# ClashLuke/LocAtE

Measured on AMD Instinct MI355X. Metric: images/sec (G+D step) 64x64 bs=64, higher is better.
Workload: dtype f32 (contractions fp32-faithful on the matrix cores: 2 x scaled fp16 operand pieces / 3 MFMAs per slice where the operand's largest magnitude comes with it, else 3 x bf16 pieces / 6 MFMAs; fp32 accumulate); 1 GPU; LocAtE G+D step, 64x64 RGB, batch 64 per GPU (the fp32 variant - the reference's own precision - of BASELINE.json configs[1]: 64x64 RGB bs 64), self/feature attention at 16x16 and 64x64, random-init weights; global_batch=64, image_size=64, parallelism=dp1, launch=hipGraph replay, G-step generator pass on a second stream

## Files before the change

locate_amd/csrc/conv.hip:

```cpp
#include "igemm.h"

template <int WGM, int WGN, int TM, int TN>
__global__ void __launch_bounds__(256) conv_igemm_kernel(const IgParams p) {
    constexpr int BK = IG_BK;
    constexpr int BM = WGM * TM * 32;
    constexpr int BN = WGN * TN * 32;
    constexpr int KPT = BK * BN / 256;
    constexpr int A_F4 = BK * BM / 4;
    constexpr int A_PT = (A_F4 + 255) / 256;
    static_assert(WGM * WGN == 4, "four waves");
    static_assert(BN % 64 == 0 && KPT == 8, "one 8-row group of the offset table per thread and step");
    static_assert(BK <= IG_TAIL, "panel tail shorter than the prefetch distance (one stage beyond the last)");

    __shared__ __attribute__((aligned(16))) float As[2][BK][BM];
    __shared__ __attribute__((aligned(16))) float Bs[2][BK][BN];

    int bx, by, bz;
    xcd_tile(bx, by, bz, p.tile_nphase);
    const int zphase = bz / p.ksplit, zsplit = bz - zphase * p.ksplit;
    const IgPhase& ph = p.ph[zphase];
    const int N = p.B * ph.QH * ph.QW;
    const int n0 = bx * BN;
    const int m0 = by * BM;
    if (n0 >= N) return;

    const int tid = threadIdx.x, lane = tid & 63, wid = tid >> 6;
    const int wm = wid / WGN, wn = wid % WGN;

    const int ncol = tid % BN;
    const int kgrp = __builtin_amdgcn_readfirstlane(tid / BN);
    const GatherCol gc = gather_setup(p, ph, n0 + ncol, N);
    float col_scale[TN];
    igemm_col_scales<WGM, WGN, TM, TN>(p, ph, col_scale, N, n0, wn, lane);

// ... 95 lines not shown
__global__ void __launch_bounds__(64 * NW, (NW == 8 ? 1 : (WGM * TM > 4 ? 2 : ((WGM * TM * TN <= IG_FOUR_BLOCKS_TILES && WGM * TM * TN >= IG_FOUR_BLOCKS_MIN && NP <= 2) ? 4 : 3)))) conv_igemm_bx6_kernel(const IgParams p) {
    constexpr int BK = 4 * NW, KB = BK / 8, KS = BK / 16, NT = 64 * NW;
    constexpr int BM = WGM * TM * 32;
    constexpr int BN = WGN * TN * 32;
    static_assert(NW == 4 || NW == 8, "four or eight waves");
    static_assert(WGM * WGN == NW, "wave grid");
    static_assert(BN == 128 && KB * BN == NT, "one gathered fragment (k-block) per thread and stage");
    static_assert(KB * BM <= 2 * NT, "at most two weight fragments per thread and stage");
    static_assert(B6_BK == 16, "the host's split-K accounting counts 16-deep steps");
    constexpr bool A2 = KB * BM > NT;
    static_assert(2 * BK <= IG_TAIL && (IG_TAIL % 8) == 0, "panel tail shorter than the prefetch distance");

    constexpr int A_U4 = 2 * NP * KB * BM, B_U4 = 2 * NP * KB * BN;
    constexpr int EPI_U4 = (NW * 32 * 33 + 8 + 3) / 4;
    constexpr int SMEM_U4 = A_U4 + B_U4 > EPI_U4 ? A_U4 + B_U4 : EPI_U4;
    __shared__ uint4 smem[SMEM_U4];
    uint4 (*As)[NP][KB][BM] = reinterpret_cast<uint4 (*)[NP][KB][BM]>(smem);
    uint4 (*Bs)[NP][KB][BN] = reinterpret_cast<uint4 (*)[NP][KB][BN]>(smem + A_U4);

    int bx, by, bz;
    xcd_tile(bx, by, bz, p.tile_nphase);
    const int zphase = bz / p.ksplit, zsplit = bz - zphase * p.ksplit;
    const IgPhase& ph = p.ph[zphase];
    const int N = p.B * ph.QH * ph.QW;
    const int n0 = bx * BN;
    const int m0 = by * BM;
    if (n0 >= N) return;

    const int tid = threadIdx.x, lane = tid & 63, wid = tid >> 6;
    const int wm = wid / WGN, wn = wid % WGN;

    const int ncol = tid % BN;
    const int kgrp = __builtin_amdgcn_readfirstlane(tid / BN);
    const GatherCol gc = gather_setup(p, ph, n0 + ncol, N);
    float col_scale[TN];
    igemm_col_scales<WGM, WGN, TM, TN>(p, ph, col_scale, N, n0, wn, lane);
    float b_scale = 1.0f, a_unscale = 1.0f, b_unscale = 1.0f;
    if constexpr (NP == 2) {
        const int kb_ = f16_scale_exp(absmax_read(p.b_absmax));
        const int ka_ = f16_scale_exp(__builtin_amdgcn_readfirstlane(*ph.a_absmax));
        b_scale = pow2f(kb_);
        unscale_pair(ka_, kb_, a_unscale, b_unscale);
    }

    f32x16 acc[TM][TN];
#pragma unroll
    for (int i = 0; i < TM; ++i)
#pragma unroll
        for (int j = 0; j < TN; ++j)
#pragma unroll
            for (int r = 0; r < 16; ++r) acc[i][j][r] = 0.0f;

    const int total_steps = ph.Kpad / BK;
    const int per_split = (total_steps + p.ksplit - 1) / p.ksplit;
    const int step0 = zsplit * per_split;
    int nsteps = total_steps - step0;
    if (nsteps > per_split) nsteps = per_split;
    if (nsteps < 0) nsteps = 0;

    const bool a_thread = KB * BM == NT || tid < KB * BM;
    const int a_kb = a_thread ? tid / BM : 0, a_m = a_thread ? tid % BM : 0;
    const uint4* ap = ph.w3 + (long long)(step0 * KB + a_kb) * ph.ld + (m0 + a_m);
    const long long a_step = (long long)KB * ph.ld, a_plane = ph.w3_plane;
    const bool b_thread = A2 && tid + NT < KB * BM;
    const int b_kb = b_thread ? (tid + NT) / BM : 0, b_m = b_thread ? (tid + NT) % BM : 0;
    const uint4* bp = ph.w3 + (long long)(step0 * KB + b_kb) * ph.ld + (m0 + b_m);
    int kidx = step0 * BK + kgrp * 8;

    uint4 areg0, areg1, areg2;
    uint4 areg3, areg4, areg5;
    float breg[8];
    i32x8 offs = *reinterpret_cast<const i32x8*>(ph.koff + __builtin_amdgcn_readfirstlane(kidx));
    unsigned long long taps = *reinterpret_cast<const unsigned long long*>(ph.ktap + __builtin_amdgcn_readfirstlane(kidx));
    auto issue_loads = [&]() {
        areg0 = ap[0];
        if constexpr (NP >= 2) areg1 = ap[a_plane];
        if constexpr (NP == 3) areg2 = ap[2 * a_plane];
        ap += a_step;
        if constexpr (A2) {
            areg3 = bp[0];
            if constexpr (NP >= 2) areg4 = bp[a_plane];
            if constexpr (NP == 3) areg5 = bp[2 * a_plane];
            bp += a_step;
        }
#pragma unroll
        for (int j = 0; j < 8; ++j) breg[j] = gather_load(gc, offs[j], (unsigned)(taps >> (8 * j)) & 31u);
        kidx += BK;
        const int ks = __builtin_amdgcn_readfirstlane(kidx);
// ... 26 lines not shown
            float v[8];
#pragma unroll
            for (int j = 0; j < 8; ++j) v[j] = breg[j];
            split3_trunc_x8(v, h, m, l);
            Bs[buf][0][kgrp][ncol] = h;
            Bs[buf][NP - 2][kgrp][ncol] = m;
            Bs[buf][NP - 1][kgrp][ncol] = l;
        } else {
            bf16x8 h;
#pragma unroll
            for (int j = 0; j < 8; ++j) h[j] = (__bf16)breg[j];
            Bs[buf][0][kgrp][ncol] = *reinterpret_cast<uint4*>(&h);
        }
    };

    if (nsteps > 0) {
        issue_loads();
        store_tiles(0);
        issue_loads();
    }
    __syncthreads();
    const int lrow = lane >> 5, lcol = lane & 31;
    constexpr int PROD = NP == 3 ? 6 : (NP == 2 ? 3 : 1);
    constexpr int NMF = TM * TN * PROD, HALF = KS == 1 ? NMF / 2 : NMF;
    using frag_t = typename std::conditional<NP == 2, f16x8, bf16x8>::type;
    for (int s = 0; s < nsteps; ++s) {
        const int buf = s & 1;
        frag_t a[TM][NP], b[TN][NP];
        auto fragments = [&](int ksub) {
#pragma unroll
            for (int i = 0; i < TM; ++i)
#pragma unroll
                for (int q = 0; q < NP; ++q) a[i][q] = *reinterpret_cast<const frag_t*>(&As[buf][q][2 * ksub + lrow][(wm * TM + i) * 32 + lcol]);
#pragma unroll
            for (int j = 0; j < TN; ++j)
// ... 107 lines not shown
                    for (int f = 0; f < HB; ++f)
                        v[zz][f] = __builtin_amdgcn_raw_buffer_load_b128(srs, (int)(t0 + (unsigned)(z0 + zz) * zstride + (unsigned)((h0 + f) * NT * 16)), 0, 16);
#pragma unroll
                for (int zz = 0; zz < ZB; ++zz)
#pragma unroll
                    for (int f = 0; f < HB; ++f) {
                        const int g = h0 + f, i = g / (TN * 4), j = (g / 4) % TN, q = g % 4;
#pragma unroll
                        for (int e = 0; e < 4; ++e) acc[i][j][4 * q + e] += __uint_as_float(v[zz][f][e]);
                    }
            }
        }
        __syncthreads();
        combined = true;
    }
    igemm_epilogue<WGM, WGN, TM, TN>(p, ph, acc, col_scale, N, n0, m0, combined ? 0 : zsplit, wm, wn, lane, stage, p.ksplit > 1 && !combined);
}

__global__ void __launch_bounds__(256) igemm_slab_reduce_kernel(const float* __restrict__ slab, float* __restrict__ out,
                                                                const float* __restrict__ bias, const float* __restrict__ scale,
                                                                int scale_bg, int scale_stride, int B, int M, int plane,
                                                                long long out_bs, long long slab_stride, int ksplit,
                                                                float* __restrict__ act_out, long long act_bs,
                                                                const float* __restrict__ mul_pre, long long mul_bs,
                                                                unsigned* __restrict__ out_absmax) {
    const unsigned per_b = (unsigned)M * (unsigned)plane;
    const unsigned total = (unsigned)B * per_b;
    const unsigned stride = gridDim.x * blockDim.x;
    const DivU32 dpb(per_b), dpl((unsigned)plane);
    float am = 0.0f;
    for (unsigned i = blockIdx.x * blockDim.x + threadIdx.x; i < total; i += stride) {
// ... 279 lines not shown
    igemm_slab_reduce_kernel<<<stream_grid(p.slab_stride, 256), 256, 0, st>>>(p.slab, p.out, p.bias, p.scale, p.scale_bg, p.scale_stride, p.B, p.M, p.OH * p.OW,
                                                                              p.out_bs, p.slab_stride, p.ksplit, p.act_out, p.act_bs, p.mul_pre, p.mul_bs, p.out_absmax);
}

template <int NP>
static void launch_bx6(const IgParams& p, dim3 grid, int bm, bool w8, hipStream_t st) {
    if (w8) {
        if (bm == 128) conv_igemm_bx6_kernel<2, 4, 2, 1, NP, 8><<<grid, 512, 0, st>>>(p);
        else conv_igemm_bx6_kernel<2, 4, 1, 1, NP, 8><<<grid, 512, 0, st>>>(p);
        return;
    }
    with_tile<true>(bm, [&](auto t) { using T = decltype(t); conv_igemm_bx6_kernel<T::wgm, T::wgn, T::tm, T::tn, NP><<<grid, 256, 0, st>>>(p); });
}

static int launch_igemm(IgParams& p, int nmax, void* slab_ws, unsigned* counters, hipStream_t st, const char* who) {
    p.tile_nphase = (path_disabled("phasefast") || (long long)p.OH * p.OW < 1024) ? 1 : p.nphase;
    if (p.win) return launch_win_igemm(p, nmax, slab_ws, counters, st, who);
    if (skinny_ok(p)) {
        p.ksplit = 1;
        launch_skinny(p, st);
        LOCATE_LAUNCH_CHECK(who);
        return LOCATE_OK;
    }
    if (pointwise_ok(p)) {
        p.ksplit = 1;
        launch_pointwise(p, st);
        LOCATE_LAUNCH_CHECK(who);
        return LOCATE_OK;
    }
    const int bm = igemm_bm(p.M, nmax, p.nphase);
// ... 442 lines not shown
```

locate_amd/csrc/convfp8.hip:

```cpp
#include "igemm.h"

__device__ __forceinline__ uint4 quant_fp8x16(const float (&v)[16], float sc) {
    unsigned w[4];
#pragma unroll
    for (int q = 0; q < 4; ++q) {
        int t = 0;
        t = __builtin_amdgcn_cvt_pk_fp8_f32(v[4 * q + 0] * sc, v[4 * q + 1] * sc, t, false);
        t = __builtin_amdgcn_cvt_pk_fp8_f32(v[4 * q + 2] * sc, v[4 * q + 3] * sc, t, true);
        w[q] = (unsigned)t;
    }
    return make_uint4(w[0], w[1], w[2], w[3]);
}

template <int WGM, int WGN, int TM, int TN>
__global__ void __launch_bounds__(256, (WGM * TM > 4 ? 2 : 3)) conv_igemm_fp8_kernel(const IgParams p) {
    constexpr int BK = 32, KB = 2, NT = 256, NW = 4;
    constexpr int BM = WGM * TM * 32;
    constexpr int BN = WGN * TN * 32;
    static_assert(WGM * WGN == NW && BN == 128 && KB * BN == NT, "one gathered chunk (16 k) per thread and stage");
    static_assert(KB * BM <= 2 * NT, "at most two weight chunks per thread and stage");
    constexpr bool A2 = KB * BM > NT;
    static_assert(2 * BK <= IG_TAIL, "panel tail shorter than the prefetch distance");
    constexpr int A_U4 = 2 * KB * BM, B_U4 = 2 * KB * BN;
    constexpr int EPI_U4 = (NW * 32 * 33 + 8 + 3) / 4;
    constexpr int SMEM_U4 = A_U4 + B_U4 > EPI_U4 ? A_U4 + B_U4 : EPI_U4;
    __shared__ uint4 smem[SMEM_U4];
    uint4 (*As)[KB][BM] = reinterpret_cast<uint4 (*)[KB][BM]>(smem);
    uint4 (*Bs)[KB][BN] = reinterpret_cast<uint4 (*)[KB][BN]>(smem + A_U4);

    int bx, by, bz;
    xcd_tile(bx, by, bz, p.tile_nphase);
    const int zphase = bz / p.ksplit, zsplit = bz - zphase * p.ksplit;
    const IgPhase& ph = p.ph[zphase];
    const int N = p.B * ph.QH * ph.QW;
    const int n0 = bx * BN;
    const int m0 = by * BM;
    if (n0 >= N) return;

    const int tid = threadIdx.x, lane = tid & 63, wid = tid >> 6;
    const int wm = wid / WGN, wn = wid % WGN;
    const int ncol = tid % BN;
    const int kgrp = __builtin_amdgcn_readfirstlane(tid / BN);
    const GatherCol gc = gather_setup(p, ph, n0 + ncol, N);
    float col_scale[TN];
    igemm_col_scales<WGM, WGN, TM, TN>(p, ph, col_scale, N, n0, wn, lane);
    const int kb_ = f8_scale_exp(absmax_read(p.b_absmax));
    const int ka_ = f8_scale_exp(__builtin_amdgcn_readfirstlane(*ph.a_absmax));
// ... 174 lines not shown
```

locate_amd/csrc/convwgrad.hip:

```cpp
#include "igemm.h"

#define WG_BK 32

struct WgParams {
    const float* x;
    const float* gy;
    float* slab;
    long long x_bs, gy_bs;
    unsigned x_bytes;
    int B, C, H, W, M, OH, OW, KH, KW, stride, pad_h, pad_w;
    int R;
    int N;
    int chunk;
    int zper, Ng;
    unsigned q_mul, ow_mul;
    int q_s1, q_s2, ow_s1, ow_s2;
    int gscale_bg, gscale_stride;
    float* direct_out;
    const float* w_ref;
    const float* inv_scale;
    double* partial;
    const unsigned* x_absmax;
    const unsigned* g_absmax;
};


template <int WGM, int WGN, int TM, int TN>
__device__ __forceinline__ void wgrad_epilogue(const WgParams& p, f32x16 (&acc)[TM][TN], int r0, int m0, int wm, int wn, int lane,
                                               int wid, int tid) {
    const int lrow = lane >> 5, lcol = lane & 31;
    __shared__ double red[4];
    const bool direct = p.direct_out != nullptr;
    float* dst = direct ? p.direct_out : p.slab + (long long)blockIdx.z * p.M * p.R;
    const float sc = (direct && p.inv_scale && p.gscale_bg == 0) ? p.inv_scale[0] : 1.0f;
    double dot = 0.0;
    const bool want_dot = direct && p.w_ref != nullptr;
#pragma unroll
    for (int j = 0; j < TN; ++j) {
        const int r = r0 + (wn * TN + j) * 32 + lcol;
// ... 17 lines not shown
                if (r_ok && m < p.M) dst[(long long)m * p.R + r] = v * sc;
            }
            dot += (double)part;
        }
    }
    if (direct && p.partial) {
        dot = wave_sum_d(dot);
        if (lane == 0) red[wid] = dot;
        __syncthreads();
        if (tid == 0) p.partial[blockIdx.y * gridDim.x + blockIdx.x] = (red[0] + red[1]) + (red[2] + red[3]);
    }
}

template <int WGM, int WGN, int TM, int TN>
__global__ void __launch_bounds__(256) conv_wgrad_kernel(const WgParams p) {
    constexpr int BM = WGM * TM * 32;
    constexpr int BR = WGN * TN * 32;
    constexpr int G_PT = WG_BK * BM / 256;
    constexpr int X_PT = WG_BK * BR / 256;
    static_assert(WGM * WGN == 4, "four waves");

    __shared__ float Gs[2][WG_BK][BM + 1];
    __shared__ float Xs[2][WG_BK][BR + 1];
    __shared__ int rt_off[BR];
    __shared__ signed char rt_dy[BR], rt_dx[BR];

    const int tid = threadIdx.x, lane = tid & 63, wid = tid >> 6;
    const int wm = wid / WGN, wn = wid % WGN;
    const int r0 = blockIdx.x * BR, m0 = blockIdx.y * BM;
    const int taps = p.KH * p.KW;
// ... 108 lines not shown
#pragma unroll
                for (int j = 0; j < TN; ++j) acc[i][j] = __builtin_amdgcn_mfma_f32_32x32x2f32(a[i], b[j], acc[i][j], 0, 0, 0);
        }
        if (s + 1 < nsteps) store_tiles(buf ^ 1);
        __syncthreads();
    }

    wgrad_epilogue<WGM, WGN, TM, TN>(p, acc, r0, m0, wm, wn, lane, wid, tid);
}

#define WB_BK 16
#define WB_PITCH 8

template <int WGM, int WGN, int TM, int TN, int NP>
__global__ void __launch_bounds__(256, (WGM * TM > 4 ? 2 : 3)) conv_wgrad_bx6_kernel(const WgParams p) {
    constexpr int BM = WGM * TM * 32;
    constexpr int BR = WGN * TN * 32;
    constexpr int G_PT = BM / 32;
    constexpr int X_PT = BR / 32;
    static_assert(WGM * WGN == 4, "four waves");

    constexpr int NPL = NP == 4 ? 1 : NP;
    __shared__ unsigned Gs[2][NPL][NP == 4 ? 1 : BM][WB_PITCH];
    __shared__ unsigned Xs[2][NPL][NP == 4 ? 1 : BR][WB_PITCH];
    __shared__ __attribute__((aligned(16))) unsigned short G8[2][NP == 4 ? BM : 1][8];
    __shared__ __attribute__((aligned(16))) unsigned short X8[2][NP == 4 ? BR : 1][8];

    const int tid = threadIdx.x, lane = tid & 63, wid = tid >> 6;
    const int wm = wid / WGN, wn = wid % WGN;
    const int r0 = blockIdx.x * BR, m0 = blockIdx.y * BM;
// ... 436 lines not shown
}

static int wgrad_reduce_zp(int nsplit, int64_t n) {
    if (nsplit >= 64 && n < knob_int("LOCATE_ZP16_MAX_N", 1 << 12)) return 16;
    return (nsplit >= 16 && n < (1 << 20)) ? 4 : 1;
}
static int wgrad_reduce_grid(int64_t n, int nsplit) {
    const int epb = 256 / wgrad_reduce_zp(nsplit, n);
    int g = stream_grid(n, epb);
    return g > 2048 ? 2048 : g;
}

struct PwParams {
    const float* x;
    const float* gy;
    float* slab;
    const float* inv_scale;
    long long x_bs, gy_bs;
    int B, C, M, P;
    int N;
    int steps, chunk;
    int tiles_c;
    int gscale_bg, gscale_stride;
    const unsigned* x_absmax;
    const unsigned* g_absmax;
};

template <int TM, int TN, int NP>
__global__ void __launch_bounds__(256) pw_wgrad_kernel(const PwParams p) {
    __shared__ float red[3][TM * TN * 16][64];
    const int lane = threadIdx.x & 63, wid = __builtin_amdgcn_readfirstlane((int)threadIdx.x >> 6);
    const int lrow = lane >> 5, lcol = lane & 31;
    const int tm = blockIdx.y / p.tiles_c, tc = blockIdx.y - tm * p.tiles_c;
    const int m0 = tm * (TM * 32), c0 = tc * (TN * 32);
    const int z = blockIdx.x * 4 + wid;
    const int s_begin = z * p.chunk;
    int s_end = s_begin + p.chunk;
    if (s_end > p.steps) s_end = p.steps;

    float gs0 = 1.0f, gs1 = 1.0f, gs2 = 1.0f, gs3 = 1.0f;
    if (p.gscale_bg > 0) {
        const int ng = p.B / p.gscale_bg;
        gs0 = p.inv_scale[0];
        gs1 = ng > 1 ? p.inv_scale[p.gscale_stride] : 1.0f;
// ... 611 lines not shown
    if (r.kind == WG_ONEPIX) {
        const OnePix op = {g.H * g.W, g.W, g.KH, g.KW, g.pad_h, g.pad_w, g.C};
        skinny_wgrad_kernel<<<r.grid, 256, 0, st>>>(x, x_bs, gy, gy_bs, gw, w_ref, inv_scale, scale_group_batch, scale_stride,
                                                   inner_partial, g.B, g.M, g.C * g.H * g.W, op);
        LOCATE_LAUNCH_CHECK("locate_conv_wgrad(one output pixel)");
        return LOCATE_OK;
    }
    const dim3 grid = r.grid;
    if (r.kind == WG_POINTWISE) {
        const PwPlan& pq = r.pw;
        LOCATE_REQUIRE((x_bs & 3) == 0 && (gy_bs & 3) == 0 &&
                       ((reinterpret_cast<uintptr_t>(x) | reinterpret_cast<uintptr_t>(gy)) & 15) == 0,
                       "locate_conv_wgrad: narrow 1x1 layers need 16-byte aligned x / gy and batch strides that are multiples of 4");
        LOCATE_REQUIRE(workspace, "locate_conv_wgrad: the split reduction needs a workspace");
        PwParams q;
        q.x = x; q.gy = gy; q.slab = static_cast<float*>(workspace); q.x_bs = x_bs; q.gy_bs = gy_bs;
        q.B = g.B; q.C = g.C; q.M = g.M; q.P = g.H * g.W; q.N = g.B * g.H * g.W; q.steps = pq.steps; q.chunk = pq.chunk;
        q.tiles_c = pq.tiles_c;
        const bool grouped = scale_group_batch > 0;
        q.inv_scale = grouped ? inv_scale : nullptr; q.gscale_bg = scale_group_batch; q.gscale_stride = scale_stride;
        const int key = (pq.tm - 1) * 2 + (pq.tn - 1);
        q.x_absmax = static_cast<const unsigned*>(x_absmax);
        q.g_absmax = static_cast<const unsigned*>(gy_absmax);
        if (precision == 2 && x_absmax && gy_absmax && !grouped) {
            if (key == 0) pw_wgrad_kernel<1, 1, 2><<<grid, 256, 0, st>>>(q);
            else if (key == 1) pw_wgrad_kernel<1, 2, 2><<<grid, 256, 0, st>>>(q);
            else if (key == 2) pw_wgrad_kernel<2, 1, 2><<<grid, 256, 0, st>>>(q);
            else pw_wgrad_kernel<2, 2, 2><<<grid, 256, 0, st>>>(q);
        } else if (precision == 1) {
            if (key == 0) pw_wgrad_kernel<1, 1, 1><<<grid, 256, 0, st>>>(q);
            else if (key == 1) pw_wgrad_kernel<1, 2, 1><<<grid, 256, 0, st>>>(q);
            else if (key == 2) pw_wgrad_kernel<2, 1, 1><<<grid, 256, 0, st>>>(q);
            else pw_wgrad_kernel<2, 2, 1><<<grid, 256, 0, st>>>(q);
        } else {
            if (key == 0) pw_wgrad_kernel<1, 1, 3><<<grid, 256, 0, st>>>(q);
            else if (key == 1) pw_wgrad_kernel<1, 2, 3><<<grid, 256, 0, st>>>(q);
            else if (key == 2) pw_wgrad_kernel<2, 1, 3><<<grid, 256, 0, st>>>(q);
            else pw_wgrad_kernel<2, 2, 3><<<grid, 256, 0, st>>>(q);
        }
        LOCATE_LAUNCH_CHECK("locate_conv_wgrad(pointwise)");
        return reduce(q.slab, grouped ? nullptr : inv_scale, "locate_conv_wgrad(pointwise reduce)");
    }
    const int bm = r.bm, nsplit = r.nsplit, chunk = r.chunk, zper = r.zper;
    LOCATE_REQUIRE(nsplit == 1 || workspace, "locate_conv_wgrad: split reduction needs a workspace");
    WgParams p;
    p.x = x; p.gy = gy; p.slab = static_cast<float*>(workspace); p.x_bs = x_bs; p.gy_bs = gy_bs;
    p.B = g.B; p.C = g.C; p.H = g.H; p.W = g.W; p.M = g.M; p.OH = g.OH; p.OW = g.OW; p.KH = g.KH; p.KW = g.KW;
    p.stride = g.stride; p.pad_h = g.pad_h; p.pad_w = g.pad_w;
    p.R = g.C * g.KH * g.KW; p.N = g.B * g.OH * g.OW; p.chunk = chunk;
    p.zper = zper; p.Ng = gd > 1 ? p.N / gd : p.N;
    fastdiv_make((unsigned)(g.OH * g.OW), &p.q_mul, &p.q_s1, &p.q_s2);
    fastdiv_make((unsigned)g.OW, &p.ow_mul, &p.ow_s1, &p.ow_s2);
    const bool direct = nsplit == 1;
    const bool grouped = scale_group_batch > 0;
    p.gscale_bg = scale_group_batch; p.gscale_stride = scale_stride;
    p.x_absmax = static_cast<const unsigned*>(x_absmax);
    p.g_absmax = static_cast<const unsigned*>(gy_absmax);
    p.direct_out = direct ? gw : nullptr;
    p.w_ref = direct ? w_ref : nullptr;
    p.inv_scale = (direct || grouped) ? inv_scale : nullptr;
// ... 43 lines not shown
```

locate_amd/csrc/convwin.hip:

```cpp
#include "igemm.h"

typedef unsigned u32x2 __attribute__((ext_vector_type(2)));
typedef int i32x2 __attribute__((ext_vector_type(2)));
typedef int i32x4 __attribute__((ext_vector_type(4)));

template <int WGM, int WGN, int TM, int TN, int NP, int SL, int BPT>
__global__ void __launch_bounds__(256, 2) conv_win_kernel(const IgParams p) {
    constexpr int NT = 256, NW = 4, U = 2 * SL;
    constexpr int BM = WGM * TM * 32;
    constexpr int BN = WGN * TN * 32;
    static_assert(WGM * WGN == NW && (BN == 128 || BN == 256), "four waves on a 128- or 256-column tile");
    constexpr int A_CH = U * BM;
    constexpr int A_PT = (A_CH + NT - 1) / NT;
    constexpr int A_U4 = 2 * NP * A_CH;
    static_assert(2 * U <= WIN_TAIL_UNITS, "panel tail shorter than the prefetch distance");

    extern __shared__ uint4 smem[];

    int bx, by, bz;
    xcd_tile(bx, by, bz, p.tile_nphase);
    const int zphase = bz / p.ksplit, zsplit = bz - zphase * p.ksplit;
    const IgPhase& ph = p.ph[zphase];
    const int QHW = ph.QH * ph.QW;
    const int N = p.B * QHW;
    const int n0 = bx * BN;
    const int m0 = by * BM;
    if (n0 >= N) return;

    const int tid = threadIdx.x, lane = tid & 63, wid = tid >> 6;
    const int wm = wid / WGN, wn = wid % WGN;
    const int lrow = lane >> 5, lcol = lane & 31;

    const int T = ph.T, Tp = ph.win_Tp, NG = ph.win_NG;
    const int WINC = Tp == 1 ? U : 1;
    const int SP = p.win_slotsp;
    const int HW = p.H * p.W;
// ... 493 lines not shown
```

locate_amd/csrc/igemm.h:

```cpp
#pragma once
#include "common.h"
#include <cstdlib>
#include <cstring>
#include <stdlib.h>
#include <type_traits>

#ifdef LOCATE_DEBUG_KNOBS
static bool path_disabled(const char* name) {
    static const char* env = getenv("LOCATE_DISABLE");
    return env != nullptr && strstr(env, name) != nullptr;
}
static int knob_int(const char* name, int fallback) {
    const char* v = getenv(name);
    return v != nullptr ? atoi(v) : fallback;
}
#else
static constexpr bool path_disabled(const char*) { return false; }
static constexpr int knob_int(const char*, int fallback) { return fallback; }
#endif

typedef float f32x16 __attribute__((ext_vector_type(16)));

#define IG_BK 16
#define IG_KPAD 32
// ... 158 lines not shown
        ll[j] = (_Float16)(x - (float)hh[j]);
    }
    h = *reinterpret_cast<uint4*>(&hh);
    l = *reinterpret_cast<uint4*>(&ll);
}

__device__ __forceinline__ void split2_f16_pair(float v0, float v1, unsigned& h, unsigned& l) {
    typedef _Float16 f16x2 __attribute__((ext_vector_type(2)));
    f16x2 hh, ll;
    hh[0] = (_Float16)v0; hh[1] = (_Float16)v1;
    ll[0] = (_Float16)(v0 - (float)hh[0]); ll[1] = (_Float16)(v1 - (float)hh[1]);
    h = *reinterpret_cast<unsigned*>(&hh);
    l = *reinterpret_cast<unsigned*>(&ll);
}

struct IgPhase {
    const float* wp;
    const int* koff;
    const unsigned char* ktap;
    const uint4* w3;
    const unsigned* a_absmax;
    long long w3_plane;
    int K, Kpad, ld, T;
    int dmin;
    int oy0, ox0, QH, QW;
    int TW, tw_magic;
    int dy0, dys, dx0, dxs;
    int win_Tp, win_NG, win_TR, win_NI, win_WR;
    unsigned win_wrw_mul;
    int win_wrw_s1, win_wrw_s2;
    int tapc[32] __attribute__((aligned(32)));
};

struct IgParams {
    const float* in;
    float* out;
    const float* bias;
    const float* scale;
    int scale_bg;
    int scale_stride;
    long long in_bs, out_bs;
    unsigned in_bytes;
    int B, C, H, W;
    int M, OH, OW;
    int istride, ostep, nphase;
    int ksplit;
    float* slab;
    long long slab_stride;
    int precision;
    const unsigned* b_absmax;
    float* act_out = nullptr;
    long long act_bs = 0;
    const float* lat = nullptr;
    long long lat_bs = 0;
    int lat_z = 0;
    const float* mul_pre = nullptr;
    long long mul_bs = 0;
    unsigned* out_absmax = nullptr;
    int combine;
    unsigned* counters;
    int tile_nphase;
    int win;
    int win_dbg;
    int win_U, win_slotsp, win_bm, win_bn;
    IgPhase ph[4];
};

template <int WGM, int WGN, int TM, int TN>
__device__ __forceinline__ void igemm_col_scales(const IgParams& p, const IgPhase& ph, float (&col_scale)[TN], int N, int n0,
                                                 int wn, int lane) {
    const int lcol = lane & 31;
#pragma unroll
    for (int j = 0; j < TN; ++j) {
        const int nj = n0 + (wn * TN + j) * 32 + lcol;
        const int nn = nj < N ? nj : 0;
        const int b = nn / (ph.QH * ph.QW);
        col_scale[j] = p.scale ? p.scale[(p.scale_bg ? b / p.scale_bg : 0) * p.scale_stride] : 1.0f;
    }
}

template <int WGM, int WGN, int TM, int TN>
__device__ __forceinline__ void igemm_epilogue(const IgParams& p, const IgPhase& ph, f32x16 (&acc)[TM][TN],
                                               const float (&col_scale)[TN], int N, int n0, int m0, int zsplit, int wm,
                                               int wn, int lane, float* stage, bool split) {
    const int lrow = lane >> 5, lcol = lane & 31;
    const long long plane = (long long)p.OH * p.OW;
    const int iplane = (int)plane;
    if (stage != nullptr && p.nphase == 1 && p.ostep == 1 && iplane <= 16 && (iplane & (iplane - 1)) == 0 &&
        ph.QH * ph.QW == iplane) {
        const int lp = __ffs(iplane) - 1;
        const bool fused_s = !split && (p.act_out != nullptr || p.mul_pre != nullptr);
        float am_s = 0.0f;
        float* out_base = split ? p.slab + (long long)zsplit * p.slab_stride : p.out;
        const long long obs = split ? (long long)p.M * plane : p.out_bs;
#pragma unroll
        for (int i = 0; i < TM; ++i) {
            const int mt0 = m0 + (wm * TM + i) * 32;
            float bias_v[16];
#pragma unroll
            for (int r = 0; r < 16; ++r) {
                const int m = mt0 + (r & 3) + 8 * (r >> 2) + 4 * lrow;
                const bool use = p.bias != nullptr && !split && m < p.M;
                const float* bp = use ? p.bias + m : p.in;
                bias_v[r] = use ? *bp : 0.0f;
            }
#pragma unroll
            for (int j = 0; j < TN; ++j) {
                const int nt0 = n0 + (wn * TN + j) * 32;
#pragma unroll
                for (int r = 0; r < 16; ++r) {
                    const int ml = (r & 3) + 8 * (r >> 2) + 4 * lrow;
                    stage[lcol * 33 + ml] = split ? acc[i][j][r] : fmaf(acc[i][j][r], col_scale[j], bias_v[r]);
                }
                __builtin_amdgcn_fence(__ATOMIC_SEQ_CST, "wavefront");
                const int b0 = nt0 >> lp;
                if (!fused_s) {
// ... 71 lines not shown
        const int b = nn / qhw, q = nn - b * qhw;
        const int qy = q / ph.QW, qx = q - qy * ph.QW;
        const long long pix = (long long)(ph.oy0 + qy * p.ostep) * p.OW + (ph.ox0 + qx * p.ostep);
        const float* o = split ? p.slab + (long long)zsplit * p.slab_stride + (long long)b * p.M * plane + pix
                               : p.out + (long long)b * p.out_bs + pix;
        optr[j] = nj < N ? o : nullptr;
        xoff[j] = (long long)b * ((p.mul_pre ? p.mul_bs : p.act_bs) - p.out_bs);
    }
    float am = 0.0f;
#pragma unroll
    for (int i = 0; i < TM; ++i) {
        float bias_v[16];
#pragma unroll
        for (int r = 0; r < 16; ++r) {
            const int m = m0 + (wm * TM + i) * 32 + (r & 3) + 8 * (r >> 2) + 4 * lrow;
            const bool use = p.bias != nullptr && !split && m < p.M;
            const float* bp = use ? p.bias + m : p.in;
            bias_v[r] = use ? *bp : 0.0f;
        }
#pragma unroll
        for (int j = 0; j < TN; ++j) {
            float* o = const_cast<float*>(optr[j]);
            if (o == nullptr) continue;
            if (!fused) {
#pragma unroll
                for (int r = 0; r < 16; ++r) {
                    const int m = m0 + (wm * TM + i) * 32 + (r & 3) + 8 * (r >> 2) + 4 * lrow;
                    if (m < p.M) o[(long long)m * plane] = split ? acc[i][j][r] : fmaf(acc[i][j][r], col_scale[j], bias_v[r]);
                }
            } else if (p.mul_pre != nullptr) {
// ... 67 lines not shown
            const int th = (t * ph.tw_magic) >> 16, tw = t - th * ph.TW;
            const bool ok = (unsigned)(iy0 + ph.dy0 + ph.dys * th) < (unsigned)p.H &&
                            (unsigned)(ix0 + ph.dx0 + ph.dxs * tw) < (unsigned)p.W;
            inside |= (ok ? 1u : 0u) << t;
        }
    }
    g.outside = ~inside;
    return g;
}

__device__ __forceinline__ float gather_load(const GatherCol& g, int soff, unsigned tap) {
    const unsigned vo = ((g.outside << (31u - tap)) & 0x80000000u) | g.lane_off;
    return __builtin_bit_cast(float, __builtin_amdgcn_raw_buffer_load_b32(g.rsrc, (int)vo, soff, 0));
}

typedef int i32x8 __attribute__((ext_vector_type(8)));
typedef unsigned u32x4 __attribute__((ext_vector_type(4)));


__device__ __forceinline__ int fastdiv(int n, unsigned mul, int s1, int s2) {
    const unsigned t = __umulhi((unsigned)n, mul);
    return (int)((t + (((unsigned)n - t) >> s1)) >> s2);
}
static void fastdiv_make(unsigned d, unsigned* mul, int* s1, int* s2) {
    if (d <= 1) { *mul = 0; *s1 = 0; *s2 = 0; return; }
    int l = 0;
    while ((1ull << l) < d) ++l;
    *mul = (unsigned)(((1ull << 32) * ((1ull << l) - d)) / d + 1);
    *s1 = 1; *s2 = l - 1;
}

// ... 19 lines not shown
```

Measured before the change: 7268 images/sec.

## Prefetch hot kernel-argument lines in bursts and stage bias in LDS early

Reorders the IgParams, IgPhase, WgParams and PwParams structs so the fields each prologue reads sit in the first one or two 64-byte lines. Each conv kernel now starts with an inline-asm burst of scalar loads that pulls those kernarg lines into the scalar cache at once, instead of taking serial misses. In the bx6 kernel, the offset/tap table and absmax reads are issued earlier; the b-absmax read is done one line per lane and reduced with DPP, and the bias is loaded once into LDS before the main loop instead of in the epilogue. This adds inline asm that depends on the struct layout and a small LDS allocation, with debug knobs to turn each piece off.

```diff
diff --git a/locate_amd/csrc/conv.hip b/locate_amd/csrc/conv.hip
--- a/locate_amd/csrc/conv.hip
+++ b/locate_amd/csrc/conv.hip
@@ -15,9 +15,11 @@
     __shared__ __attribute__((aligned(16))) float As[2][BK][BM];
     __shared__ __attribute__((aligned(16))) float Bs[2][BK][BN];
 
+    if (!HOT_ARGS_LAZY(p)) hot_args_burst<true>();
     int bx, by, bz;
     xcd_tile(bx, by, bz, p.tile_nphase);
     const int zphase = bz / p.ksplit, zsplit = bz - zphase * p.ksplit;
+    if (zphase > 0 && !HOT_ARGS_LAZY(p)) hot_phase_burst<2>(zphase);
     const IgPhase& ph = p.ph[zphase];
     const int N = p.B * ph.QH * ph.QW;
     const int n0 = bx * BN;
@@ -143,13 +145,18 @@
     constexpr int A_U4 = 2 * NP * KB * BM, B_U4 = 2 * NP * KB * BN;
     constexpr int EPI_U4 = (NW * 32 * 33 + 8 + 3) / 4;
     constexpr int SMEM_U4 = A_U4 + B_U4 > EPI_U4 ? A_U4 + B_U4 : EPI_U4;
-    __shared__ uint4 smem[SMEM_U4];
+    __shared__ uint4 smem[SMEM_U4 + BM / 4];
     uint4 (*As)[NP][KB][BM] = reinterpret_cast<uint4 (*)[NP][KB][BM]>(smem);
     uint4 (*Bs)[NP][KB][BN] = reinterpret_cast<uint4 (*)[NP][KB][BN]>(smem + A_U4);
-
+    float* const bias_s = reinterpret_cast<float*>(smem + SMEM_U4);
+
+    constexpr bool HOT_OK = !(NP == 1 && NW == 4 && WGM * TM * TN == 1);
+    const bool hot = HOT_OK && !HOT_EARLY_OFF(p), hot_bias = HOT_OK && !HOT_BIAS_OFF(p), hot_burst = HOT_OK && !HOT_ARGS_LAZY(p);
+    if (hot_burst) hot_args_burst<true>();
     int bx, by, bz;
     xcd_tile(bx, by, bz, p.tile_nphase);
     const int zphase = bz / p.ksplit, zsplit = bz - zphase * p.ksplit;
+    if (zphase > 0 && hot_burst) hot_phase_burst<2>(zphase);
     const IgPhase& ph = p.ph[zphase];
     const int N = p.B * ph.QH * ph.QW;
     const int n0 = bx * BN;
@@ -161,24 +168,6 @@
 
     const int ncol = tid % BN;
     const int kgrp = __builtin_amdgcn_readfirstlane(tid / BN);
-    const GatherCol gc = gather_setup(p, ph, n0 + ncol, N);
-    float col_scale[TN];
-    igemm_col_scales<WGM, WGN, TM, TN>(p, ph, col_scale, N, n0, wn, lane);
-    float b_scale = 1.0f, a_unscale = 1.0f, b_unscale = 1.0f;
-    if constexpr (NP == 2) {
-        const int kb_ = f16_scale_exp(absmax_read(p.b_absmax));
-        const int ka_ = f16_scale_exp(__builtin_amdgcn_readfirstlane(*ph.a_absmax));
-        b_scale = pow2f(kb_);
-        unscale_pair(ka_, kb_, a_unscale, b_unscale);
-    }
-
-    f32x16 acc[TM][TN];
-#pragma unroll
-    for (int i = 0; i < TM; ++i)
-#pragma unroll
-        for (int j = 0; j < TN; ++j)
-#pragma unroll
-            for (int r = 0; r < 16; ++r) acc[i][j][r] = 0.0f;
 
     const int total_steps = ph.Kpad / BK;
     const int per_split = (total_steps + p.ksplit - 1) / p.ksplit;
@@ -186,6 +175,37 @@
     int nsteps = total_steps - step0;
     if (nsteps > per_split) nsteps = per_split;
     if (nsteps < 0) nsteps = 0;
+    int kidx = step0 * BK + kgrp * 8;
+
+    i32x8 offs;
+    unsigned long long taps;
+    unsigned b_word = 0, a_word = 0;
+    if (hot) {
+        offs = *reinterpret_cast<const i32x8*>(ph.koff + __builtin_amdgcn_readfirstlane(kidx));
+        taps = *reinterpret_cast<const unsigned long long*>(ph.ktap + __builtin_amdgcn_readfirstlane(kidx));
+        if constexpr (NP == 2) {
+            b_word = p.b_absmax[AMAX_STRIDE * (tid & (AMAX_LINES - 1))];
+            a_word = *ph.a_absmax;
+        }
+    }
+    const GatherCol gc = gather_setup(p, ph, n0 + ncol, N);
+    float col_scale[TN];
+    igemm_col_scales<WGM, WGN, TM, TN>(p, ph, col_scale, N, n0, wn, lane);
+    float b_scale = 1.0f, a_unscale = 1.0f, b_unscale = 1.0f;
+    if constexpr (NP == 2) {
+        const int kb_ = f16_scale_exp(hot ? absmax_reduce_dpp(b_word) : absmax_read(p.b_absmax));
+        const int ka_ = f16_scale_exp(__builtin_amdgcn_readfirstlane(hot ? a_word : *ph.a_absmax));
+        b_scale = pow2f(kb_);
+        unscale_pair(ka_, kb_, a_unscale, b_unscale);
+    }
+
+    f32x16 acc[TM][TN];
+#pragma unroll
+    for (int i = 0; i < TM; ++i)
+#pragma unroll
+        for (int j = 0; j < TN; ++j)
+#pragma unroll
+            for (int r = 0; r < 16; ++r) acc[i][j][r] = 0.0f;
 
     const bool a_thread = KB * BM == NT || tid < KB * BM;
     const int a_kb = a_thread ? tid / BM : 0, a_m = a_thread ? tid % BM : 0;
@@ -194,13 +214,14 @@
     const bool b_thread = A2 && tid + NT < KB * BM;
     const int b_kb = b_thread ? (tid + NT) / BM : 0, b_m = b_thread ? (tid + NT) % BM : 0;
     const uint4* bp = ph.w3 + (long long)(step0 * KB + b_kb) * ph.ld + (m0 + b_m);
-    int kidx = step0 * BK + kgrp * 8;
 
     uint4 areg0, areg1, areg2;
     uint4 areg3, areg4, areg5;
     float breg[8];
-    i32x8 offs = *reinterpret_cast<const i32x8*>(ph.koff + __builtin_amdgcn_readfirstlane(kidx));
-    unsigned long long taps = *reinterpret_cast<const unsigned long long*>(ph.ktap + __builtin_amdgcn_readfirstlane(kidx));
+    if (!hot) {
+        offs = *reinterpret_cast<const i32x8*>(ph.koff + __builtin_amdgcn_readfirstlane(kidx));
+        taps = *reinterpret_cast<const unsigned long long*>(ph.ktap + __builtin_amdgcn_readfirstlane(kidx));
+    }
     auto issue_loads = [&]() {
         areg0 = ap[0];
         if constexpr (NP >= 2) areg1 = ap[a_plane];
@@ -257,11 +278,19 @@
         }
     };
 
+    float bias_r = 0.0f;
+    static_assert(BM <= NT, "one bias row per thread");
+    if (hot_bias) {
+        const bool use = p.bias != nullptr && tid < BM && m0 + tid < p.M;
+        const float* bp_ = use ? p.bias + (m0 + tid) : p.in;
+        bias_r = use ? *bp_ : 0.0f;
+    }
     if (nsteps > 0) {
         issue_loads();
         store_tiles(0);
         issue_loads();
     }
+    if (hot_bias && tid < BM) bias_s[tid] = bias_r;
     __syncthreads();
     const int lrow = lane >> 5, lcol = lane & 31;
     constexpr int PROD = NP == 3 ? 6 : (NP == 2 ? 3 : 1);
@@ -399,7 +428,8 @@
         __syncthreads();
         combined = true;
     }
-    igemm_epilogue<WGM, WGN, TM, TN>(p, ph, acc, col_scale, N, n0, m0, combined ? 0 : zsplit, wm, wn, lane, stage, p.ksplit > 1 && !combined);
+    igemm_epilogue<WGM, WGN, TM, TN>(p, ph, acc, col_scale, N, n0, m0, combined ? 0 : zsplit, wm, wn, lane, stage, p.ksplit > 1 && !combined,
+                                     hot_bias ? bias_s : nullptr);
 }
 
 __global__ void __launch_bounds__(256) igemm_slab_reduce_kernel(const float* __restrict__ slab, float* __restrict__ out,
@@ -709,6 +739,7 @@
 }
 
 static int launch_igemm(IgParams& p, int nmax, void* slab_ws, unsigned* counters, hipStream_t st, const char* who) {
+    p.lazy = (path_disabled("hotargs") ? 7 : 0) | (path_disabled("hotburst") ? 1 : 0) | (path_disabled("hotearly") ? 2 : 0) | (path_disabled("hotbias") ? 4 : 0);
     p.tile_nphase = (path_disabled("phasefast") || (long long)p.OH * p.OW < 1024) ? 1 : p.nphase;
     if (p.win) return launch_win_igemm(p, nmax, slab_ws, counters, st, who);
     if (skinny_ok(p)) {
diff --git a/locate_amd/csrc/convfp8.hip b/locate_amd/csrc/convfp8.hip
--- a/locate_amd/csrc/convfp8.hip
+++ b/locate_amd/csrc/convfp8.hip
@@ -28,9 +28,11 @@
     uint4 (*As)[KB][BM] = reinterpret_cast<uint4 (*)[KB][BM]>(smem);
     uint4 (*Bs)[KB][BN] = reinterpret_cast<uint4 (*)[KB][BN]>(smem + A_U4);
 
+    if (!HOT_ARGS_LAZY(p)) hot_args_burst<true>();
     int bx, by, bz;
     xcd_tile(bx, by, bz, p.tile_nphase);
     const int zphase = bz / p.ksplit, zsplit = bz - zphase * p.ksplit;
+    if (zphase > 0 && !HOT_ARGS_LAZY(p)) hot_phase_burst<2>(zphase);
     const IgPhase& ph = p.ph[zphase];
     const int N = p.B * ph.QH * ph.QW;
     const int n0 = bx * BN;
diff --git a/locate_amd/csrc/convwgrad.hip b/locate_amd/csrc/convwgrad.hip
--- a/locate_amd/csrc/convwgrad.hip
+++ b/locate_amd/csrc/convwgrad.hip
@@ -2,27 +2,35 @@
 
 #define WG_BK 32
 
-struct WgParams {
+struct alignas(64) WgParams {
     const float* x;
     const float* gy;
-    float* slab;
     long long x_bs, gy_bs;
+    const unsigned* x_absmax;
+    const unsigned* g_absmax;
+    const float* inv_scale;
     unsigned x_bytes;
-    int B, C, H, W, M, OH, OW, KH, KW, stride, pad_h, pad_w;
+    int B, H, W, M, OH, OW, KH, KW, stride, pad_h, pad_w;
     int R;
-    int N;
     int chunk;
     int zper, Ng;
+    int gscale_bg, gscale_stride;
     unsigned q_mul, ow_mul;
     int q_s1, q_s2, ow_s1, ow_s2;
-    int gscale_bg, gscale_stride;
+    int C;
+    int N;
+    float* slab;
     float* direct_out;
     const float* w_ref;
-    const float* inv_scale;
     double* partial;
-    const unsigned* x_absmax;
-    const unsigned* g_absmax;
+#ifdef LOCATE_DEBUG_KNOBS
+    int lazy;
+#endif
 };
+static_assert(offsetof(WgParams, x) == 0 && offsetof(WgParams, q_mul) == 128, "WgParams: the hot block is the first two 64-byte lines");
+#ifndef LOCATE_DEBUG_KNOBS
+static_assert(sizeof(WgParams) == 192, "WgParams must not grow");
+#endif
 
 
 template <int WGM, int WGN, int TM, int TN>
@@ -70,6 +78,7 @@
 
 template <int WGM, int WGN, int TM, int TN>
 __global__ void __launch_bounds__(256) conv_wgrad_kernel(const WgParams p) {
+    if (!HOT_ARGS_LAZY(p)) flat_args_burst<192>();
     constexpr int BM = WGM * TM * 32;
     constexpr int BR = WGN * TN * 32;
     constexpr int G_PT = WG_BK * BM / 256;
@@ -208,6 +217,9 @@
 
 template <int WGM, int WGN, int TM, int TN, int NP>
 __global__ void __launch_bounds__(256, (WGM * TM > 4 ? 2 : 3)) conv_wgrad_bx6_kernel(const WgParams p) {
+    if constexpr (!(NP == 1 && WGM * TM * TN == 1)) {
+        if (!HOT_ARGS_LAZY(p)) flat_args_burst<192>();
+    }
     constexpr int BM = WGM * TM * 32;
     constexpr int BR = WGN * TN * 32;
     constexpr int G_PT = BM / 32;
@@ -674,20 +686,30 @@
 struct PwParams {
     const float* x;
     const float* gy;
-    float* slab;
     const float* inv_scale;
+    const unsigned* x_absmax;
+    const unsigned* g_absmax;
     long long x_bs, gy_bs;
     int B, C, M, P;
     int N;
     int steps, chunk;
     int tiles_c;
     int gscale_bg, gscale_stride;
-    const unsigned* x_absmax;
-    const unsigned* g_absmax;
+    float* slab;
+#ifdef LOCATE_DEBUG_KNOBS
+    int lazy;
+#endif
 };
+static_assert(offsetof(PwParams, slab) == 96, "PwParams: everything the prologue reads leads");
+#ifndef LOCATE_DEBUG_KNOBS
+static_assert(sizeof(PwParams) == 104, "PwParams must not grow");
+#endif
 
 template <int TM, int TN, int NP>
 __global__ void __launch_bounds__(256) pw_wgrad_kernel(const PwParams p) {
+    if constexpr (!((NP == 1 && TM * TN == 2) || (NP == 3 && TN == 1))) {
+        if (!HOT_ARGS_LAZY(p)) flat_args_burst<104>();
+    }
     __shared__ float red[3][TM * TN * 16][64];
     const int lane = threadIdx.x & 63, wid = __builtin_amdgcn_readfirstlane((int)threadIdx.x >> 6);
     const int lrow = lane >> 5, lcol = lane & 31;
@@ -1329,6 +1351,9 @@
                        "locate_conv_wgrad: narrow 1x1 layers need 16-byte aligned x / gy and batch strides that are multiples of 4");
         LOCATE_REQUIRE(workspace, "locate_conv_wgrad: the split reduction needs a workspace");
         PwParams q;
+#ifdef LOCATE_DEBUG_KNOBS
+        q.lazy = path_disabled("hotargs") ? 1 : 0;
+#endif
         q.x = x; q.gy = gy; q.slab = static_cast<float*>(workspace); q.x_bs = x_bs; q.gy_bs = gy_bs;
         q.B = g.B; q.C = g.C; q.M = g.M; q.P = g.H * g.W; q.N = g.B * g.H * g.W; q.steps = pq.steps; q.chunk = pq.chunk;
         q.tiles_c = pq.tiles_c;
@@ -1359,6 +1384,9 @@
     const int bm = r.bm, nsplit = r.nsplit, chunk = r.chunk, zper = r.zper;
     LOCATE_REQUIRE(nsplit == 1 || workspace, "locate_conv_wgrad: split reduction needs a workspace");
     WgParams p;
+#ifdef LOCATE_DEBUG_KNOBS
+    p.lazy = path_disabled("hotargs") ? 1 : 0;
+#endif
     p.x = x; p.gy = gy; p.slab = static_cast<float*>(workspace); p.x_bs = x_bs; p.gy_bs = gy_bs;
     p.B = g.B; p.C = g.C; p.H = g.H; p.W = g.W; p.M = g.M; p.OH = g.OH; p.OW = g.OW; p.KH = g.KH; p.KW = g.KW;
     p.stride = g.stride; p.pad_h = g.pad_h; p.pad_w = g.pad_w;
diff --git a/locate_amd/csrc/convwin.hip b/locate_amd/csrc/convwin.hip
--- a/locate_amd/csrc/convwin.hip
+++ b/locate_amd/csrc/convwin.hip
@@ -17,9 +17,11 @@
 
     extern __shared__ uint4 smem[];
 
+    if (!HOT_ARGS_LAZY(p)) hot_args_burst<true>();
     int bx, by, bz;
     xcd_tile(bx, by, bz, p.tile_nphase);
     const int zphase = bz / p.ksplit, zsplit = bz - zphase * p.ksplit;
+    if (!HOT_ARGS_LAZY(p)) hot_phase_burst<5>(zphase);
     const IgPhase& ph = p.ph[zphase];
     const int QHW = ph.QH * ph.QW;
     const int N = p.B * QHW;
diff --git a/locate_amd/csrc/igemm.h b/locate_amd/csrc/igemm.h
--- a/locate_amd/csrc/igemm.h
+++ b/locate_amd/csrc/igemm.h
@@ -1,5 +1,6 @@
 #pragma once
 #include "common.h"
+#include <cstddef>
 #include <cstdlib>
 #include <cstring>
 #include <stdlib.h>
@@ -196,6 +197,7 @@
     l = *reinterpret_cast<unsigned*>(&ll);
 }
 
+#define IG_PHASE_HOT 96
 struct IgPhase {
     const float* wp;
     const int* koff;
@@ -203,50 +205,133 @@
     const uint4* w3;
     const unsigned* a_absmax;
     long long w3_plane;
-    int K, Kpad, ld, T;
+    int Kpad, ld, T;
     int dmin;
-    int oy0, ox0, QH, QW;
+    int QH, QW;
     int TW, tw_magic;
     int dy0, dys, dx0, dxs;
+    int K;
+    int oy0, ox0;
     int win_Tp, win_NG, win_TR, win_NI, win_WR;
     unsigned win_wrw_mul;
     int win_wrw_s1, win_wrw_s2;
     int tapc[32] __attribute__((aligned(32)));
 };
 
-struct IgParams {
+#define IG_HOT 128
+struct alignas(64) IgParams {
     const float* in;
     float* out;
     const float* bias;
     const float* scale;
-    int scale_bg;
-    int scale_stride;
+    const unsigned* b_absmax;
     long long in_bs, out_bs;
     unsigned in_bytes;
+    int scale_bg, scale_stride;
     int B, C, H, W;
     int M, OH, OW;
     int istride, ostep, nphase;
     int ksplit;
+    int tile_nphase;
+    int combine;
+    int win_U, win_slotsp;
     float* slab;
     long long slab_stride;
-    int precision;
-    const unsigned* b_absmax;
     float* act_out = nullptr;
     long long act_bs = 0;
+    const float* mul_pre = nullptr;
+    long long mul_bs = 0;
+    unsigned* out_absmax = nullptr;
+    unsigned* counters;
     const float* lat = nullptr;
     long long lat_bs = 0;
     int lat_z = 0;
-    const float* mul_pre = nullptr;
-    long long mul_bs = 0;
-    unsigned* out_absmax = nullptr;
-    int combine;
-    unsigned* counters;
-    int tile_nphase;
+    int precision;
     int win;
     int win_dbg;
-    int win_U, win_slotsp, win_bm, win_bn;
+    int win_bm, win_bn;
+    int lazy = 0;
     IgPhase ph[4];
 };
+static_assert(offsetof(IgParams, in) == 0 && offsetof(IgParams, slab) == IG_HOT, "IgParams: the hot block is the first two 64-byte lines");
+static_assert(offsetof(IgParams, lat) == IG_HOT + 64, "IgParams: the epilogue's fields are line 2");
+static_assert(offsetof(IgPhase, wp) == 0 && offsetof(IgPhase, K) == IG_PHASE_HOT, "IgPhase: the hot block leads");
+static_assert(offsetof(IgParams, ph) % 32 == 0 && sizeof(IgPhase) % 32 == 0 && IG_PHASE_HOT <= 96,
+              "IgPhase: a hot block of <= 96 bytes that starts on a 32-byte boundary lies inside two 64-byte lines");
+static_assert(sizeof(IgPhase) <= 288 && sizeof(IgParams) <= 1408, "the records must not grow");
+
+typedef int i32x8 __attribute__((ext_vector_type(8)));
+template <bool HIDDEN>
+__device__ __forceinline__ void hot_args_burst() {
+    const auto ka = __builtin_amdgcn_kernarg_segment_ptr();
+    int t0, t1, t2, t3, t4, t5;
+    constexpr int PH = (int)offsetof(IgParams, ph);
+    static_assert(PH % 64 == 0 && sizeof(IgParams) % 64 == 0 && IG_PHASE_HOT <= 128, "line-aligned blocks");
+    if constexpr (HIDDEN) {
+        asm volatile("s_load_dword %0, %6, 0x0\n\ts_load_dword %1, %6, %9\n\ts_load_dword %2, %6, 0x40\n\t"
+                     "s_load_dword %3, %6, %7\n\ts_load_dword %4, %6, %8\n\ts_load_dword %5, %6, 0x80\n\t"
+                     "s_waitcnt lgkmcnt(0)"
+                     : "=&s"(t0), "=&s"(t1), "=&s"(t2), "=&s"(t3), "=&s"(t4), "=&s"(t5)
+                     : "s"(ka), "i"(PH), "i"(PH + 64), "i"((int)sizeof(IgParams)) : "memory");
+    } else {
+        asm volatile("s_load_dword %0, %5, 0x0\n\ts_load_dword %1, %5, 0x40\n\t"
+                     "s_load_dword %2, %5, %6\n\ts_load_dword %3, %5, %7\n\ts_load_dword %4, %5, 0x80\n\t"
+                     "s_waitcnt lgkmcnt(0)"
+                     : "=&s"(t0), "=&s"(t1), "=&s"(t2), "=&s"(t3), "=&s"(t4) : "s"(ka), "i"(PH), "i"(PH + 64) : "memory");
+    }
+}
+template <int LINES>
+__device__ __forceinline__ void hot_phase_burst(int zphase) {
+    static_assert(LINES == 2 || LINES == 5, "hot block, or the whole phase record");
+    static_assert(((offsetof(IgParams, ph) + 3 * sizeof(IgPhase)) & ~(size_t)63) + 5 * 64 <= sizeof(IgParams), "the burst stays inside the record");
+    const auto ka = __builtin_amdgcn_kernarg_segment_ptr();
+    const int o = __builtin_amdgcn_readfirstlane(((int)offsetof(IgParams, ph) + zphase * (int)sizeof(IgPhase)) & ~63);
+    const int o1 = o + 64;
+    int t0, t1;
+    if constexpr (LINES == 2) {
+        asm volatile("s_nop 4\n\ts_load_dword %0, %2, %3\n\ts_load_dword %1, %2, %4\n\ts_waitcnt lgkmcnt(0)"
+                     : "=&s"(t0), "=&s"(t1) : "s"(ka), "s"(o), "s"(o1) : "memory");
+    } else {
+        const int o2 = o + 128, o3 = o + 192, o4 = o + 256;
+        int t2, t3, t4;
+        asm volatile("s_nop 4\n\ts_load_dword %0, %5, %6\n\ts_load_dword %1, %5, %7\n\ts_load_dword %2, %5, %8\n\t"
+                     "s_load_dword %3, %5, %9\n\ts_load_dword %4, %5, %10\n\ts_waitcnt lgkmcnt(0)"
+                     : "=&s"(t0), "=&s"(t1), "=&s"(t2), "=&s"(t3), "=&s"(t4) : "s"(ka), "s"(o), "s"(o1), "s"(o2), "s"(o3), "s"(o4) : "memory");
+    }
+}
+template <int BYTES>
+__device__ __forceinline__ void flat_args_burst() {
+    static_assert(BYTES == 192 || BYTES == 104, "WgParams or PwParams");
+    const auto ka = __builtin_amdgcn_kernarg_segment_ptr();
+    int t0, t1;
+    if constexpr (BYTES == 192) {
+        int t2;
+        asm volatile("s_load_dword %0, %3, 0x0\n\ts_load_dword %1, %3, 0x40\n\ts_load_dword %2, %3, 0x80\n\ts_waitcnt lgkmcnt(0)"
+                     : "=&s"(t0), "=&s"(t1), "=&s"(t2) : "s"(ka) : "memory");
+    } else {
+        asm volatile("s_load_dword %0, %2, 0x0\n\ts_load_dword %1, %2, 0x40\n\ts_waitcnt lgkmcnt(0)"
+                     : "=&s"(t0), "=&s"(t1) : "s"(ka) : "memory");
+    }
+}
+__device__ __forceinline__ unsigned absmax_reduce_dpp(unsigned v) {
+    static_assert(AMAX_LINES == 32, "two rows of sixteen lanes");
+    int x = (int)v, w;
+    w = __builtin_amdgcn_update_dpp(x, x, 0xB1, 0xf, 0xf, false); x = (unsigned)w > (unsigned)x ? w : x;
+    w = __builtin_amdgcn_update_dpp(x, x, 0x4E, 0xf, 0xf, false); x = (unsigned)w > (unsigned)x ? w : x;
+    w = __builtin_amdgcn_update_dpp(x, x, 0x141, 0xf, 0xf, false); x = (unsigned)w > (unsigned)x ? w : x;
+    w = __builtin_amdgcn_update_dpp(x, x, 0x140, 0xf, 0xf, false); x = (unsigned)w > (unsigned)x ? w : x;
+    const unsigned r0 = (unsigned)__builtin_amdgcn_readlane(x, 0), r1 = (unsigned)__builtin_amdgcn_readlane(x, 16);
+    return r0 > r1 ? r0 : r1;
+}
+#ifdef LOCATE_DEBUG_KNOBS
+#define HOT_ARGS_LAZY(p) (((p).lazy & 1) != 0)
+#define HOT_EARLY_OFF(p) (((p).lazy & 2) != 0)
+#define HOT_BIAS_OFF(p) (((p).lazy & 4) != 0)
+#else
+#define HOT_ARGS_LAZY(p) false
+#define HOT_EARLY_OFF(p) false
+#define HOT_BIAS_OFF(p) false
+#endif
 
 template <int WGM, int WGN, int TM, int TN>
 __device__ __forceinline__ void igemm_col_scales(const IgParams& p, const IgPhase& ph, float (&col_scale)[TN], int N, int n0,
@@ -264,7 +349,7 @@
 template <int WGM, int WGN, int TM, int TN>
 __device__ __forceinline__ void igemm_epilogue(const IgParams& p, const IgPhase& ph, f32x16 (&acc)[TM][TN],
                                                const float (&col_scale)[TN], int N, int n0, int m0, int zsplit, int wm,
-                                               int wn, int lane, float* stage, bool split) {
+                                               int wn, int lane, float* stage, bool split, const float* bias_s = nullptr) {
     const int lrow = lane >> 5, lcol = lane & 31;
     const long long plane = (long long)p.OH * p.OW;
     const int iplane = (int)plane;
@@ -282,6 +367,7 @@
 #pragma unroll
             for (int r = 0; r < 16; ++r) {
                 const int m = mt0 + (r & 3) + 8 * (r >> 2) + 4 * lrow;
+                if (bias_s != nullptr) { bias_v[r] = split ? 0.0f : bias_s[m - m0]; continue; }
                 const bool use = p.bias != nullptr && !split && m < p.M;
                 const float* bp = use ? p.bias + m : p.in;
                 bias_v[r] = use ? *bp : 0.0f;
@@ -383,6 +469,7 @@
 #pragma unroll
         for (int r = 0; r < 16; ++r) {
             const int m = m0 + (wm * TM + i) * 32 + (r & 3) + 8 * (r >> 2) + 4 * lrow;
+            if (bias_s != nullptr) { bias_v[r] = split ? 0.0f : bias_s[m - m0]; continue; }
             const bool use = p.bias != nullptr && !split && m < p.M;
             const float* bp = use ? p.bias + m : p.in;
             bias_v[r] = use ? *bp : 0.0f;
@@ -480,7 +567,6 @@
     return __builtin_bit_cast(float, __builtin_amdgcn_raw_buffer_load_b32(g.rsrc, (int)vo, soff, 0));
 }
 
-typedef int i32x8 __attribute__((ext_vector_type(8)));
 typedef unsigned u32x4 __attribute__((ext_vector_type(4)));
 
 
```

New measurement: 6928 images/sec. -4.7%, worse.
